# A-SHOJAEI/preference-guided-image-captioning-alignment

Measured on AMD Instinct MI355X. Metric: DPO preference-pairs/sec, CLIP-ViT-B/32+GPT-2-M seq128, higher is better.
Workload: dtype bf16; 1 GPU; Stage-2 DPO step, 4-forward policy/reference x chosen/rejected, openai/clip-vit-base-patch32 (frozen) + gpt2-medium decoder, seq_len 128, beta 0.1, bf16 MFMA / f32 accumulate+master, AdamW+clip; pairs_per_gpu=512, seq_len=128, parallelism=dp1, grad_allreduce=none (1 GPU)

## Files before the change

include/pgca_hip.h:

```cpp
#ifndef PGCA_HIP_H
#define PGCA_HIP_H

#include <stddef.h>
#include <stdint.h>

#ifdef __cplusplus
extern "C" {
#endif

typedef enum pgca_status {
  PGCA_OK = 0,
  PGCA_ERR_INVALID = -1,
  PGCA_ERR_LAUNCH = -2
} pgca_status;

#define PGCA_ABI_VERSION 306
int pgca_version(void);
int pgca_sizeof_gemm_args(void);
const char* pgca_last_error(void);

enum { PGCA_NT = 0, PGCA_NN = 1, PGCA_TN = 2 };

enum {
  PGCA_EPI_NONE = 0,
// ... 20 lines not shown
  int32_t epilogue;
  float alpha;
  const float* bias;
  void* out_bf16;
  int32_t ld_out_bf16;
  float* out_f32;
  int32_t ld_out_f32;
  int32_t accumulate;
  const float* residual;
  int32_t ld_res;
  void* aux_out;
  const void* aux_in;
  int32_t ld_aux;
  const int64_t* targets;
  float* stat_max;
  float* stat_sum;
  int32_t stat_ld;
  float* target_val;
  const float* row_lse;
  const float* row_scale;
  int32_t out_cols;
  uint32_t drop_seed;
  uint32_t drop_threshold;
  float drop_scale;
  float* colsum_part;
  int32_t ld_colsum;
  const int32_t* drop_rows;
} pgca_gemm_args;

int pgca_gemm_bf16(const pgca_gemm_args* args, void* stream);
int pgca_gemm_plan(const pgca_gemm_args* args);
int pgca_set_option(const char* name, int32_t value);
int pgca_gemm_bf16_grouped(const pgca_gemm_args* args, int32_t count, void* stream);

#define PGCA_SKINNY_MAX_M 64
typedef struct pgca_skinny_args {
  const void* x;
  const void* W;
  int32_t M, N, K, lda, ldw;
  float* scratch;
  const float* bias;
  int32_t act;
  const float* residual;
  int32_t ld_res;
  float* out_f32;
  int32_t ld_out_f32;
  void* out_bf16;
  int32_t ld_out_bf16;
  const float* ln_gamma;
  const float* ln_beta;
  float ln_eps;
  void* ln_out_bf16;
  int32_t ld_ln;
} pgca_skinny_args;
int pgca_gemm_skinny(const pgca_skinny_args* args, void* stream);
int64_t pgca_gemm_skinny_workspace(int32_t M, int32_t N, int32_t K);
int pgca_sizeof_skinny_args(void);

int pgca_rowstats_combine(const float* stat_max, const float* stat_sum, int32_t stat_ld, int32_t nparts,
                          const float* target_val, int32_t M, float* lse, float* out_logprob, void* stream);

int pgca_layernorm_fwd(const float* x, const int32_t* row_map, int32_t M, int32_t H, const float* gamma,
                       const float* beta, float eps, void* y_bf16, float* y_f32, float* mean, float* rstd,
                       void* stream);

int pgca_layernorm_bwd_blocks(int32_t M);
// ... 134 lines not shown
```

preference-guided-image-captioning-alignment_amd/csrc/gemm.hip:

```cpp
#include <string>

#include "gemm_device.h"

namespace {

template <int LA, int LB>
__global__ __launch_bounds__(256, 2) void gemm_kernel(const pgca_gemm_args a, int ntm, int ntn) {
  __shared__ __attribute__((aligned(16))) unsigned char smem[2][2][TILE_BYTES];

  int tm, tn;
  group_m_tile(xcd_remap(blockIdx.x, ntm * ntn), ntm, ntn, tm, tn);
  const int m0 = tm * BM, n0 = tn * BN;

  const int t = threadIdx.x;
  const int lane = t & 63, wave = t >> 6;
  const int wm = wave >> 1, wn = wave & 1;

  const bf16_t* A = reinterpret_cast<const bf16_t*>(a.A);
  const bf16_t* B = reinterpret_cast<const bf16_t*>(a.B);

  Stage<LA> sa;
  Stage<LB> sb;
  sa.init(t, a.lda, m0, LA == 0 ? a.M : ((a.M + 7) & ~7));
  sb.init(t, a.ldb, n0, LB == 0 ? a.N : ((a.N + 7) & ~7));
  const bf16_t* abase = LA == 0 ? A + (size_t)m0 * a.lda : A + m0;
  const bf16_t* bbase = LB == 0 ? B + (size_t)n0 * a.ldb : B + n0;
  const size_t astep = LA == 0 ? (size_t)BK : (size_t)BK * a.lda;
  const size_t bstep = LB == 0 ? (size_t)BK : (size_t)BK * a.ldb;

  f32x4 acc[4][4];
#pragma unroll
  for (int i = 0; i < 4; ++i)
#pragma unroll
    for (int j = 0; j < 4; ++j) acc[i][j] = (f32x4){0.f, 0.f, 0.f, 0.f};

// ... 27 lines not shown
        for (int j = 0; j < 4; ++j)
          acc[i][j] = __builtin_amdgcn_mfma_f32_16x16x32_bf16(fa[i], fb[j], acc[i][j], 0, 0, 0);
    }
    if (more) {
      sa.store(smem[cur ^ 1][0], ra);
      sb.store(smem[cur ^ 1][1], rb);
    }
    __syncthreads();
  }

  run_epilogue(a, acc, &smem[0][0][0], m0 + wm * 64, n0 + wn * 64, lane, wave);
}

__global__ void rowstats_combine_kernel(const float* __restrict__ smax, const float* __restrict__ ssum, int stat_ld,
                                        int nparts, const float* __restrict__ tval, int M, float* __restrict__ lse,
                                        float* __restrict__ out_lp) {
  const int row = blockIdx.x * (blockDim.x >> 6) + (threadIdx.x >> 6);
  const int lane = threadIdx.x & 63;
  if (row >= M) return;
  float mx = -INFINITY;
  for (int i = lane; i < nparts; i += 64) mx = fmaxf(mx, smax[(size_t)row * stat_ld + i]);
  mx = wave_max(mx);
  float s = 0.f;
  for (int i = lane; i < nparts; i += 64) {
    const float pm = smax[(size_t)row * stat_ld + i];
    if (pm > -INFINITY) s += ssum[(size_t)row * stat_ld + i] * __expf(pm - mx);
  }
  s = wave_sum(s);
  if (lane == 0) {
    const float l = mx + __logf(s);
    if (lse) lse[row] = l;
    if (out_lp) out_lp[row] = tval[row] - l;
  }
}


template <int LA, int LB, bool RAW = false>
__device__ __forceinline__ void gemm256_body(const pgca_gemm_args& a, int ntm, int ntn, int nk_per_split, int bid_in,
                                             int ksplit, unsigned char* smem2) {
  int tm, tn;
  if (RAW) {
    tm = bid_in / ntn;
    tn = bid_in - tm * ntn;
  } else {
    group_m_tile(xcd_remap(bid_in, ntm * ntn), ntm, ntn, tm, tn);
  }
  const int m0 = tm * BM2, n0 = tn * BN2;

  const int t = threadIdx.x;
  const int lane = t & 63;
  const int wave = __builtin_amdgcn_readfirstlane(t >> 6);
  const int wm = wave >> 2, wn = wave & 3;

  const bf16_t* A = reinterpret_cast<const bf16_t*>(a.A);
  const bf16_t* B = reinterpret_cast<const bf16_t*>(a.B);

  Dma<LA, BK> da;
  Dma<LB, BK> db;
  da.init(lane, wave, a.lda, m0, LA == 0 ? a.M : ((a.M + 7) & ~7));
  db.init(lane, wave, a.ldb, n0, LB == 0 ? a.N : ((a.N + 7) & ~7));
  const bf16_t* abase = LA == 0 ? A + (size_t)m0 * a.lda : A + m0;
  const bf16_t* bbase = LB == 0 ? B + (size_t)n0 * a.ldb : B + n0;
  const size_t astep = LA == 0 ? (size_t)BK : (size_t)BK * a.lda;
  const size_t bstep = LB == 0 ? (size_t)BK : (size_t)BK * a.ldb;

  f32x4 acc[2][4][4];
#pragma unroll
  for (int h = 0; h < 2; ++h)
#pragma unroll
    for (int i = 0; i < 4; ++i)
#pragma unroll
      for (int j = 0; j < 4; ++j) acc[h][i][j] = (f32x4){0.f, 0.f, 0.f, 0.f};

  const int kt0 = ksplit * nk_per_split;
  const int nk = min(nk_per_split, a.K / BK - kt0);
  abase += (size_t)kt0 * astep;
  bbase += (size_t)kt0 * bstep;
#ifdef PGCA_GEMM_TIMING
  unsigned long long ts0, ts1, ts2, ts3;
#endif
  TSTAMP(ts0);
  da.issue(abase, smem2, wave);
  db.issue(bbase, smem2 + TILE2_BYTES, wave);
  dma_wait();
  __syncthreads();
  TSTAMP(ts1);

  for (int kt = 0; kt < nk; ++kt) {
    const int cur = kt & 1;
    if (kt + 1 < nk) {
      unsigned char* nxt = smem2 + (cur ^ 1) * 2 * TILE2_BYTES;
      da.issue(abase + (size_t)(kt + 1) * astep, nxt, wave);
      db.issue(bbase + (size_t)(kt + 1) * bstep, nxt + TILE2_BYTES, wave);
    }
    const unsigned char* la = smem2 + cur * 2 * TILE2_BYTES;
    const unsigned char* lb = la + TILE2_BYTES;
#pragma unroll
    for (int kk = 0; kk < 2; ++kk) {
      bf16x8 fb[4];
#pragma unroll
      for (int j = 0; j < 4; ++j) fb[j] = read_frag<LB, 512>(lb, wn * 64, j, kk, lane);
      mma_half<LA>(la, wm * 128, kk, lane, fb, acc[0]);
      mma_half<LA>(la, wm * 128 + 64, kk, lane, fb, acc[1]);
    }
    dma_wait();
    __syncthreads();
  }

  TSTAMP(ts2);
  run_epilogue(a, acc[0], smem2, m0 + wm * 128, n0 + wn * 64, lane, wave);
  run_epilogue(a, acc[1], smem2, m0 + wm * 128 + 64, n0 + wn * 64, lane, wave);
#ifdef PGCA_GEMM_TIMING
  dma_wait();
  TSTAMP(ts3);
  if (a.stat_max && a.epilogue != PGCA_EPI_ROWSTATS && lane == 0) {
    float* o = a.stat_max + ((size_t)blockIdx.x * 8 + wave) * 8;
    o[0] = (float)(ts1 - ts0); o[1] = (float)(ts2 - ts1); o[2] = (float)(ts3 - ts2); o[3] = (float)nk;
  }
#endif
}

template <int LA, int LB>
__global__ __launch_bounds__(512, 2) void gemm256_kernel(const pgca_gemm_args a, int ntm, int ntn, int nk_per_split) {
  extern __shared__ __attribute__((aligned(16))) unsigned char smem2[];
  gemm256_body<LA, LB>(a, ntm, ntn, nk_per_split, blockIdx.x, blockIdx.y, smem2);
}

struct pgca_group_param {
  pgca_gemm_args a[4];
  int start[5];
  int ntm[4], ntn[4];
};

__global__ __launch_bounds__(512, 2) void gemm256_group_tn_kernel(const pgca_group_param gp) {
  extern __shared__ __attribute__((aligned(16))) unsigned char smem2[];
  const int b = xcd_remap(blockIdx.x, gp.start[4]);
  int p = 0;
  if (b >= gp.start[1]) p = 1;
  if (b >= gp.start[2]) p = 2;
  if (b >= gp.start[3]) p = 3;
#define PGCA_SEL(F) (p == 0 ? gp.a[0].F : p == 1 ? gp.a[1].F : p == 2 ? gp.a[2].F : gp.a[3].F)
  pgca_gemm_args a = {};
  a.A = PGCA_SEL(A);
  a.B = PGCA_SEL(B);
  a.M = PGCA_SEL(M);
  a.N = PGCA_SEL(N);
  a.K = PGCA_SEL(K);
  a.lda = PGCA_SEL(lda);
  a.ldb = PGCA_SEL(ldb);
  a.out_f32 = PGCA_SEL(out_f32);
  a.ld_out_f32 = PGCA_SEL(ld_out_f32);
  a.alpha = PGCA_SEL(alpha);
  a.accumulate = PGCA_SEL(accumulate);
  a.layout = PGCA_TN;
  a.epilogue = PGCA_EPI_NONE;
#undef PGCA_SEL
  const int ntm = p == 0 ? gp.ntm[0] : p == 1 ? gp.ntm[1] : p == 2 ? gp.ntm[2] : gp.ntm[3];
  const int ntn = p == 0 ? gp.ntn[0] : p == 1 ? gp.ntn[1] : p == 2 ? gp.ntn[2] : gp.ntn[3];
  const int st = p == 0 ? gp.start[0] : p == 1 ? gp.start[1] : p == 2 ? gp.start[2] : gp.start[3];
  const int l = b - st;
  int tm, tn;
  if (ntm <= ntn) {
    tn = l / ntm;
    tm = l - tn * ntm;
  } else {
    tm = l / ntn;
    tn = l - tm * ntn;
  }
  gemm256_body<1, 1, true>(a, ntm, ntn, a.K / BK, tm * ntn + tn, 0, smem2);
}

constexpr size_t GEMM256_LDS = 4 * TILE2_BYTES;

int plan_variant(const pgca_gemm_args& a) {
  const int forced = gemm_tuning().schedule;
  if (forced >= 0) return forced == 6 ? 6 : 0;
  return a.layout == PGCA_TN ? 0 : 6;
}

}

namespace pgca {
GemmTuning& gemm_tuning() {
  static GemmTuning t = [] {
    auto env = [](const char* name, int dflt) {
      const char* e = getenv(name);
      return e ? atoi(e) : dflt;
    };
    GemmTuning v;
    v.tile = env("PGCA_GEMM_TILE", 0);
    v.schedule = env("PGCA_GEMM_RING", -1);
    v.group = env("PGCA_GEMM_NO_GROUP", 0) ? 0 : 1;
    v.stagger = env("PGCA_GEMM_STAGGER", 0);
    v.pair_order = 0;
    return v;
  }();
  return t;
}

GemmPlan plan_gemm(const pgca_gemm_args& a) {
  GemmPlan p;
  p.ncols = a.epilogue == PGCA_EPI_DLOGITS ? a.out_cols : a.N;
  const int ntm2 = (a.M + BM2 - 1) / BM2, ntn2 = (p.ncols + BN2 - 1) / BN2;
  const int force = gemm_tuning().tile;
  const int nk_total = a.K / BK;
  int splits = 1;
// ... 151 lines not shown
    const pgca_gemm_args& a = args[i];
    groupable = a.layout == PGCA_TN && (a.K % BK) == 0 && a.M >= 8 && a.N >= 8 && a.epilogue == PGCA_EPI_NONE &&
                a.out_f32 && !a.out_bf16 && !a.bias && !a.residual && !a.drop_threshold &&
                check_gemm_args(a) == PGCA_OK;
  }
  if (!groupable) {
    for (int i = 0; i < count; ++i) {
      const int rc = pgca_gemm_bf16(&args[i], stream);
      if (rc) return rc;
    }
    return PGCA_OK;
  }
  if (raise_lds_limit<gemm256_group_tn_kernel>(GEMM256_LDS, "gemm256")) return PGCA_ERR_LAUNCH;
  pgca_group_param gp;
  int total = 0;
  for (int i = 0; i < 4; ++i) {
    if (i < count) {
      gp.a[i] = args[i];
      gp.ntm[i] = (args[i].M + BM2 - 1) / BM2;
      gp.ntn[i] = (args[i].N + BN2 - 1) / BN2;
      gp.start[i] = total;
      total += gp.ntm[i] * gp.ntn[i];
    } else {
      gp.a[i] = args[count - 1];
      gp.ntm[i] = gp.ntn[i] = 1;
      gp.start[i] = 0x7fffffff;
    }
  }
  gp.start[4] = total;
  hipLaunchKernelGGL(gemm256_group_tn_kernel, dim3(total), dim3(512), GEMM256_LDS, (hipStream_t)stream, gp);
  return check_launch("pgca_gemm_bf16_grouped");
}

extern "C" int pgca_rowstats_combine(const float* stat_max, const float* stat_sum, int32_t stat_ld, int32_t nparts,
                                     const float* target_val, int32_t M, float* lse, float* out_logprob,
                                     void* stream) {
  if (!stat_max || !stat_sum || M <= 0 || nparts <= 0 || (out_logprob && !target_val)) {
    set_error("pgca_rowstats_combine: bad arguments");
    return PGCA_ERR_INVALID;
  }
  hipLaunchKernelGGL(rowstats_combine_kernel, dim3((M + 3) / 4), dim3(256), 0, (hipStream_t)stream, stat_max,
                     stat_sum, stat_ld, nparts, target_val, M, lse, out_logprob);
  return check_launch("pgca_rowstats_combine");
}
```

preference-guided-image-captioning-alignment_amd/csrc/gemm_device.h:

```cpp
#pragma once
#include <stdlib.h>

#include <type_traits>

#include "common.h"

namespace pgca {
struct GemmPlan {
  int tile;
  int variant;
  int splits;
  int ntm, ntn;
  int nk_per_split;
  int grid_y;
  int ncols;
};
GemmPlan plan_gemm(const pgca_gemm_args& a);
int launch_gemm256s(const pgca_gemm_args& a, const GemmPlan& p, void* stream);
int launch_gemm256s_pair(const pgca_gemm_args& a0, const pgca_gemm_args& a1, const GemmPlan& p, void* stream);

struct GemmTuning {
  int tile;
  int schedule;
  int group;
  int pair_order;
  int stagger;
};
GemmTuning& gemm_tuning();
}

using namespace pgca;

namespace {

template <typename F>
int with_layout(int layout, F&& f) {
  using S0 = std::integral_constant<int, 0>;
  using S1 = std::integral_constant<int, 1>;
  switch (layout) {
    case PGCA_NT: return f(S0{}, S0{});
    case PGCA_NN: return f(S0{}, S1{});
    case PGCA_TN: return f(S1{}, S1{});
    default: set_error("pgca_gemm_bf16: unknown layout %d", layout); return PGCA_ERR_INVALID;
  }
}

template <auto KERNEL>
int raise_lds_limit(size_t bytes, const char* what) {
  static const bool ok = hipFuncSetAttribute((const void*)KERNEL, hipFuncAttributeMaxDynamicSharedMemorySize,
                                             (int)bytes) == hipSuccess;
  if (!ok) {
    (void)hipGetLastError();
// ... 178 lines not shown
```

preference-guided-image-captioning-alignment_amd/csrc/gemm_pair.hip:

```cpp
#include "gemm_phase_body.h"

namespace {

struct pgca_pair_param {
  pgca_gemm_args a[2];
  int ntm, ntn, nk, stagger;
  int order;
};

template <int LA, int LB>
__global__ __launch_bounds__(512, 2) void gemm256s_pair_kernel(const pgca_pair_param gp) {
  extern __shared__ __attribute__((aligned(16))) unsigned char smems[];
  const int ntm = gp.ntm, ntn = gp.ntn, nwg = ntm * ntn;
  const int b = xcd_remap(blockIdx.x, 2 * nwg);
  int p, bid;
  if (gp.order == 0) {
    p = b >= nwg;
    bid = b - (p ? nwg : 0);
  } else {
    const int per_group = GROUP_M * ntn;
    const int g = b / (2 * per_group);
    const int size = min(GROUP_M, ntm - g * GROUP_M) * ntn;
    const int rem = b - g * 2 * per_group;
    p = rem >= size;
    bid = g * per_group + rem - (p ? size : 0);
  }
  p = __builtin_amdgcn_readfirstlane(p);
  bid = __builtin_amdgcn_readfirstlane(bid);
  const char* kernarg = (const char*)__builtin_amdgcn_kernarg_segment_ptr();
  const pgca_gemm_args a = *(const pgca_gemm_args*)(kernarg + offsetof(pgca_pair_param, a) +
                                                    (p ? sizeof(pgca_gemm_args) : 0));
  if (a.epilogue > PGCA_EPI_TANH && a.epilogue != PGCA_EPI_GELU_NEW_D) return;
  gemm256s_body<LA, LB>(a, ntm, ntn, gp.nk, gp.stagger, bid, smems);
}

}

int pgca::launch_gemm256s_pair(const pgca_gemm_args& a0, const pgca_gemm_args& a1, const GemmPlan& p, void* stream) {
  auto forward_epilogue = [](int e) { return (e >= PGCA_EPI_NONE && e <= PGCA_EPI_TANH) || e == PGCA_EPI_GELU_NEW_D; };
  if (!forward_epilogue(a0.epilogue) || !forward_epilogue(a1.epilogue)) {
    const int rc = launch_gemm256s(a0, p, stream);
    return rc ? rc : launch_gemm256s(a1, p, stream);
  }
  pgca_pair_param gp;
  gp.a[0] = a0;
  gp.a[1] = a1;
  gp.ntm = p.ntm;
  gp.ntn = p.ntn;
  gp.nk = p.nk_per_split;
  gp.stagger = 2 * p.ntm * p.ntn >= 3 * 256 ? gemm_tuning().stagger : 0;
  gp.order = gemm_tuning().pair_order;
  auto launch = [&](auto lb) {
    constexpr auto kernel = gemm256s_pair_kernel<0, decltype(lb)::value>;
    if (raise_lds_limit<kernel>(GEMM256S_LDS, "gemm256s pair")) return (int)PGCA_ERR_LAUNCH;
    hipLaunchKernelGGL(kernel, dim3(2 * p.ntm * p.ntn), dim3(512), GEMM256S_LDS, (hipStream_t)stream, gp);
    return check_launch("pgca_gemm_bf16_grouped(256 phase-staggered pair)");
  };
  return a0.layout == PGCA_NT ? launch(std::integral_constant<int, 0>{}) : launch(std::integral_constant<int, 1>{});
}
```

preference-guided-image-captioning-alignment_amd/csrc/gemm_phase.hip:

```cpp
#include "gemm_phase_body.h"

namespace {

template <int LA, int LB>
__global__ __launch_bounds__(512, 2) void gemm256s_kernel(const pgca_gemm_args a, int ntm, int ntn, int nk_per_split,
                                                          int stagger) {
  extern __shared__ __attribute__((aligned(16))) unsigned char smems[];
  gemm256s_body<LA, LB>(a, ntm, ntn, nk_per_split, stagger, xcd_remap(blockIdx.x, ntm * ntn), smems);
}

}

int pgca::launch_gemm256s(const pgca_gemm_args& a, const GemmPlan& p, void* stream) {
  return with_layout(a.layout, [&](auto la, auto lb) {
    constexpr auto kernel = gemm256s_kernel<decltype(la)::value, decltype(lb)::value>;
    if (raise_lds_limit<kernel>(GEMM256S_LDS, "gemm256s")) return (int)PGCA_ERR_LAUNCH;
    const int stagger = (p.ntm * p.ntn >= 3 * 256 && p.grid_y == 1) ? gemm_tuning().stagger : 0;
    hipLaunchKernelGGL(kernel, dim3(p.ntm * p.ntn, p.grid_y), dim3(512), GEMM256S_LDS, (hipStream_t)stream, a, p.ntm,
                       p.ntn, p.nk_per_split, stagger);
    return check_launch("pgca_gemm_bf16(256 phase-staggered)");
  });
}
```

preference-guided-image-captioning-alignment_amd/csrc/gemm_phase_body.h:

```cpp
#pragma once
#include <stddef.h>

#include "gemm_device.h"

namespace {

constexpr int PBK = 32, PSTAGES = 4;
constexpr int PTILE_BYTES = 256 * PBK * 2;

template <int KS>
using DmaP = Dma<KS, PBK>;

template <int KS>
__device__ __forceinline__ bf16x8 read_frag_p(const unsigned char* lds, int wbase, int sub, int lane) {
  if (KS == 0) {
    const int row = wbase + sub * 16 + (lane & 15);
    const int pos = (lane >> 4) ^ swz4p((lane >> 2) & 3);
    return *reinterpret_cast<const bf16x8*>(lds + row * 64 + pos * 16);
  } else {
    return read_frag<1, 512>(lds, wbase, sub, 0, lane);
  }
}


template <int N>
__device__ __forceinline__ void wait_vm_p() {
  asm volatile("s_waitcnt vmcnt(%0)" ::"n"(N) : "memory");
}

#ifndef PGCA_FILL_L
#define PGCA_FILL_L 0
#endif
#ifndef PGCA_FILL_M
#define PGCA_FILL_M 0
#endif
template <int N>
__device__ __forceinline__ void valu_fill(float (&d)[8]) {
#pragma unroll
  for (int i = 0; i < N; ++i) asm volatile("v_fmac_f32 %0, %1, %1" : "+v"(d[i & 7]) : "v"(d[(i + 3) & 7]));
}
#define PGCA_PBAR()                       \
  do {                                    \
    __builtin_amdgcn_sched_barrier(0);    \
    __builtin_amdgcn_s_barrier();         \
    __builtin_amdgcn_sched_barrier(0);    \
  } while (0)

template <int LA, int LB>
__device__ __forceinline__ void gemm256s_body(const pgca_gemm_args& a, int ntm, int ntn, int nk_per_split, int stagger,
                                              int bid, unsigned char* smems) {
#ifdef PGCA_GEMM_TIMING
  unsigned long long ts0, ts1, ts2, ts3, tr0, tr3;
#endif
  TSTAMP(ts0);
  TSTAMP_REAL(tr0);

  if (stagger > 0 && gridDim.y == 1 && blockIdx.x < 256) {
    const int slot = (blockIdx.x >> 3) & 3;
    for (int i = 0; i < slot * stagger; ++i) __builtin_amdgcn_s_sleep(16);
  }

  int tm, tn;
  group_m_tile(bid, ntm, ntn, tm, tn);
  const int m0 = tm * BM2, n0 = tn * BN2;

  const int t = threadIdx.x;
  const int lane = t & 63;
  const int wave = __builtin_amdgcn_readfirstlane(t >> 6);
  const int wm = wave >> 2, wn = wave & 3;

  const bf16_t* A = reinterpret_cast<const bf16_t*>(a.A);
  const bf16_t* B = reinterpret_cast<const bf16_t*>(a.B);

  DmaP<LA> da;
  DmaP<LB> db;
  da.init(lane, wave, a.lda, m0, LA == 0 ? a.M : ((a.M + 7) & ~7));
  db.init(lane, wave, a.ldb, n0, LB == 0 ? a.N : ((a.N + 7) & ~7));
  const bf16_t* abase = LA == 0 ? A + (size_t)m0 * a.lda : A + m0;
  const bf16_t* bbase = LB == 0 ? B + (size_t)n0 * a.ldb : B + n0;
  const size_t astep = LA == 0 ? (size_t)PBK : (size_t)PBK * a.lda;
  const size_t bstep = LB == 0 ? (size_t)PBK : (size_t)PBK * a.ldb;

  f32x4 acc[2][4][4];
#pragma unroll
  for (int h = 0; h < 2; ++h)
#pragma unroll
    for (int i = 0; i < 4; ++i)
#pragma unroll
      for (int j = 0; j < 4; ++j) acc[h][i][j] = (f32x4){0.f, 0.f, 0.f, 0.f};

  const int kt0 = blockIdx.y * nk_per_split * 2;
  const int nk = min(nk_per_split * 2, a.K / PBK - kt0);
  abase += (size_t)kt0 * astep;
  bbase += (size_t)kt0 * bstep;

  da.issue(abase, smems, wave);
  db.issue(bbase, smems + PTILE_BYTES, wave);
  da.issue(abase + astep, smems + 2 * PTILE_BYTES, wave);
  db.issue(bbase + bstep, smems + 3 * PTILE_BYTES, wave);
  if (2 < nk) {
    da.issue(abase + 2 * astep, smems + 4 * PTILE_BYTES, wave);
    wait_vm_p<6>();
  } else {
    wait_vm_p<4>();
  }
  PGCA_PBAR();
  PGCA_PBAR();
  if (wm == 1) PGCA_PBAR();

  TSTAMP(ts1);
#ifdef PGCA_GEMM_TIMING2
  unsigned long long q0 = 0, q1 = 0, q2 = 0, q3 = 0, q4 = 0, q5 = 0, q6 = 0, q7 = 0, q8 = 0;
  unsigned long long aL0 = 0, aB1 = 0, aM0 = 0, aB2 = 0, aL1 = 0, aB3 = 0, aM1 = 0, aB4 = 0;
#endif
  float fill[8] = {1.f, 2.f, 3.f, 4.f, 5.f, 6.f, 7.f, 8.f};
  for (int kt = 0; kt < nk; ++kt) {
    PSTAMP(q0);
    const unsigned char* la = smems + (kt & 3) * 2 * PTILE_BYTES;
    const unsigned char* lb = la + PTILE_BYTES;
    bf16x8 fa[4], fb[4];
#pragma unroll
    for (int j = 0; j < 4; ++j) fb[j] = read_frag_p<LB>(lb, wn * 64, j, lane);
#pragma unroll
    for (int i = 0; i < 4; ++i) fa[i] = read_frag_p<LA>(la, wm * 128, i, lane);
// ... 89 lines not shown
```

preference-guided-image-captioning-alignment_amd/engine.py:

```python
from __future__ import annotations

import logging
import math
import os
from contextlib import contextmanager
from dataclasses import dataclass
from types import SimpleNamespace
from typing import Dict, List, Optional, Tuple

import torch

from . import hip
from .arch import GptArch, ModelArch, VitArch
from .params import ParamStore, Segment, VOCAB_TILE

logger = logging.getLogger(__name__)

F32, BF16, I32, I64 = torch.float32, torch.bfloat16, torch.int32, torch.int64
ATTN_BWD_MAX_S = 1024
ATTN_BWD_ONEPASS_MAX_S = 512


def attention_backward(qkv, out, dout, lse, key_mask, B, S, heads, causal, dqkv, drop=None, cu=None):
    fn = hip.attention_bwd if S <= ATTN_BWD_ONEPASS_MAX_S else hip.attention_bwd_split
# ... 1004 lines not shown
            torch.cuda.synchronize()
        return out

    def decode_reorder(self, src: torch.Tensor) -> None:
        self.trunk.decode_reorder(self._dec, src)

    def _decode_logits(self, x: torch.Tensor) -> torch.Tensor:
        a, st = self.arch.gpt, self._dec
        R, H = st.R, a.hidden
        self.trunk.decode_step(x, st, st.t)
        if st.lnf_done:
            hf = self.trunk._buf("gen.y", (R, H), BF16)
        else:
            hf = self._buf("gen.hf", (R, H), BF16)
            hip.layernorm_fwd(x, R, H, self.trunk.lnf_w.w, self.trunk.lnf_b.w, a.eps, y_bf16=hf)
        ldv = (self.V + 3) // 4 * 4
        out = self._buf("gen.logits", (R, ldv), F32)
        hip.gemm(hf, self.wte.b, R, self.V, H, hip.NT, out_f32=out, ld_out_f32=ldv)
        return out[:, :self.V]

    def backward(self, dseq: torch.Tensor) -> torch.Tensor:
        s = self.saved
        sb: SeqBatch = s["sb"]
        a = self.arch.gpt
        H, Pd, Bq, S, Mc = a.hidden, self.arch.proj_dim, sb.Bq, sb.S, sb.n_rows
        pack: Optional[RowPack] = s["pack"]
        rw = _rows(pack, Bq, S)
        M = rw.M
        ws = self.ws
        rs = self._buf("row_scale", (Mc,), F32)
        hip.row_scale(dseq, sb.seq_of_row, sb.counts, Mc, (1 if s["reduce"] == "mean" else 0) | 2, rs)
        dhf = self._buf("dhf32", (Mc, H), F32, zero=True)
        ck = min(self.LM_CHUNK, Mc)
        dl = self._buf("dlogits", (ck, self.Vp), BF16)
        for r0 in range(0, Mc, ck):
            n = min(ck, Mc - r0)
            hfc = s["hf"][r0:r0 + n]
            hip.gemm(hfc, self.wte.b, n, self.V, H, hip.NT, epilogue=hip.EPI_DLOGITS, targets=sb.targets[r0:r0 + n],
                     row_lse=s["lse"][r0:r0 + n], row_scale=rs[r0:r0 + n], out_bf16=dl, ld_out_bf16=self.Vp,
                     out_cols=self.Vp)
            hip.gemm(dl, self.wte_pad_bf, n, H, self.Vp, hip.NN, lda=self.Vp, ldb=H, out_f32=dhf[r0:r0 + n], accumulate=True)
            hip.gemm(dl, hfc, self.V, H, n, hip.TN, lda=self.Vp, ldb=H, out_f32=self.wte.g, accumulate=True)
        g = self.trunk._buf("g_top", (M, H), F32, zero=True)
        g_bf = self.trunk._buf("gbf_top", (M, H), BF16, zero=True)
        nb = hip.layernorm_bwd_blocks(Mc)
        part = ws.get("ln_part_f", (2, nb, H), F32)
        hip.layernorm_bwd(s["hL"], Mc, H, self.trunk.lnf_w.w, s["mf"], s["rf"], g, dy_f32=dhf,
                          row_map=sb.row_map_packed if pack is not None else sb.row_map, dx_bf16=g_bf, part=part,
                          drop_dx=self.trunk.top_drop(), drop_rows=rw.ids)
        _ln_param_grads(part, nb, H, self.trunk.lnf_w.g, self.trunk.lnf_b.g)
        g0 = self.trunk.backward(g, g_bf)
        drop = s["drop"]
        XH = self.arch.xattn_heads
        dh = H // XH
        datt = self._buf("datt", (Bq, H), F32, zero=True)
        nbe = hip.embed_bwd_blocks(Bq, S)
        parte = ws.get("ln_part_e", (2, nbe, H), F32)
        dvv = self._buf("dvv", (Bq, H), BF16)
        if drop is None:
            hip.embed_bwd(g0, sb.ids, sb.mask, Bq, S, H, self.wte.g, self.wpe.g, wte=self.wte.w, attended=s["att"],
                          gamma=self.anw.w, mean=s["m0"], rstd=s["r0"], dattended=datt, part=parte, cu=rw.cu)
            _ln_param_grads(parte, nbe, H, self.anw.g, self.anb.g)
            datt_bf = self._buf("datt_bf", (Bq, H), BF16)
            hip.cast_bf16(datt, datt_bf, Bq * H)
            hip.gemm(datt_bf, s["vv"], H, H, Bq, hip.TN, lda=H, ldb=H, out_f32=self.ow.g, accumulate=True)
            _bias_grad(ws, Bq, H, H, self.ob.g, x_f32=datt)
            hip.gemm(datt_bf, self.ow.b, Bq, H, H, hip.NN, out_bf16=dvv)
        else:
            dU = self._buf("dU", (Bq, XH, H), F32, zero=True)
            hip.embed_bwd(g0, sb.ids, sb.mask, Bq, S, H, self.wte.g, self.wpe.g, wte=self.wte.w, attended=self.ob.w,
                          att_stride=0, gamma=self.anw.w, mean=s["m0"], rstd=s["r0"], dattended=datt, part=parte,
                          U=s["U"], dU=dU, xheads=XH, drop_x=drop(0, KIND_XATTN), drop_e=drop(0, KIND_EMBD), cu=rw.cu)
            _ln_param_grads(parte, nbe, H, self.anw.g, self.anb.g)
            _bias_grad(ws, Bq, H, H, self.ob.g, x_f32=datt)
            dU_bf = self._buf("dU_bf", (Bq, XH, H), BF16)
# ... 180 lines not shown
```

preference-guided-image-captioning-alignment_amd/hip.py:

```python
from __future__ import annotations

import ctypes as C
import os
from typing import Optional

import torch

_HERE = os.path.dirname(os.path.abspath(__file__))
LIB_PATH = os.environ.get("PGCA_LIB") or os.path.join(_HERE, "libpgca_hip.so")

NT, NN, TN = 0, 1, 2
EPI_NONE, EPI_GELU_NEW, EPI_QUICK_GELU, EPI_RELU, EPI_TANH = 0, 1, 2, 3, 4
EPI_DGELU_NEW, EPI_DRELU, EPI_DTANH, EPI_ROWSTATS, EPI_DLOGITS, EPI_DQUICK_GELU = 5, 6, 7, 8, 9, 10
EPI_GELU_NEW_D, EPI_MUL_AUX = 11, 12

_vp, _i32, _i64, _f32 = C.c_void_p, C.c_int32, C.c_int64, C.c_float


class GemmArgs(C.Structure):
    _fields_ = [
        ("A", _vp), ("B", _vp),
        ("M", _i32), ("N", _i32), ("K", _i32),
        ("lda", _i32), ("ldb", _i32),
        ("layout", _i32), ("epilogue", _i32),
# ... 7 lines not shown
        ("targets", _vp), ("stat_max", _vp), ("stat_sum", _vp), ("stat_ld", _i32),
        ("target_val", _vp), ("row_lse", _vp), ("row_scale", _vp),
        ("out_cols", _i32),
        ("drop_seed", C.c_uint32), ("drop_threshold", C.c_uint32), ("drop_scale", _f32),
        ("colsum_part", _vp), ("ld_colsum", _i32),
        ("drop_rows", _vp),
    ]


class SkinnyArgs(C.Structure):
    _fields_ = [
        ("x", _vp), ("W", _vp),
        ("M", _i32), ("N", _i32), ("K", _i32), ("lda", _i32), ("ldw", _i32),
        ("scratch", _vp), ("bias", _vp), ("act", _i32),
        ("residual", _vp), ("ld_res", _i32),
        ("out_f32", _vp), ("ld_out_f32", _i32),
        ("out_bf16", _vp), ("ld_out_bf16", _i32),
        ("ln_gamma", _vp), ("ln_beta", _vp), ("ln_eps", _f32),
        ("ln_out_bf16", _vp), ("ld_ln", _i32),
    ]


class SelectOpts(C.Structure):
    _fields_ = [("no_repeat_ngram_size", _i32), ("n_ban", _i32), ("ban_ids", _vp)]


SKINNY_MAX_M = 64

_SIGS = {
    "pgca_gemm_bf16": [C.POINTER(GemmArgs), _vp],
    "pgca_gemm_plan": [C.POINTER(GemmArgs)],
    "pgca_set_option": [C.c_char_p, _i32],
    "pgca_gemm_bf16_grouped": [C.POINTER(GemmArgs), _i32, _vp],
    "pgca_gemm_skinny": [C.POINTER(SkinnyArgs), _vp],
    "pgca_rowstats_combine": [_vp, _vp, _i32, _i32, _vp, _i32, _vp, _vp, _vp],
    "pgca_layernorm_fwd": [_vp, _vp, _i32, _i32, _vp, _vp, _f32, _vp, _vp, _vp, _vp, _vp],
    "pgca_layernorm_bwd_blocks": [_i32],
    "pgca_layernorm_bwd": [_vp, _vp, _vp, _vp, _i32, _i32, _vp, _vp, _vp, _vp, _vp, _vp, _vp, _vp, _vp, _vp, _vp, _vp],
    "pgca_colsum_finish": [_vp, _i32, _i32, _vp, _i32, _vp],
    "pgca_colsum_finish4": [_vp, _i32, _i32, _i32, _vp, _vp, _vp, _vp, _i32, _vp],
    "pgca_colsum_blocks": [_i32],
    "pgca_colsum": [_vp, _vp, _i32, _i32, _i32, _vp, _vp],
    "pgca_attention_fwd": [_vp, _vp, _i32, _i32, _i32, _i32, _vp, _vp, C.c_uint32, C.c_uint32, _f32, _vp, _vp],
    "pgca_attention_bwd": [_vp, _vp, _vp, _vp, _vp, _i32, _i32, _i32, _i32, _vp, C.c_uint32, C.c_uint32, _f32, _vp, _vp],
    "pgca_attention_bwd_split": [_vp, _vp, _vp, _vp, _vp, _i32, _i32, _i32, _i32, _vp, C.c_uint32, C.c_uint32, _f32, _vp,
                                 _vp],
    "pgca_embed_fwd": [_vp, _i32, _i32, _i32, _vp, _vp, _vp, _vp, _vp, _f32, _vp, _vp, _vp, _i32, _vp, _i32, _vp, _vp,
                       _vp, _i32, _vp],
    "pgca_embed_bwd": [_vp, _vp, _vp, _i32, _i32, _i32, _vp, _vp, _vp, _vp, _vp, _vp, _vp, _vp, _vp, _i32, _vp, _vp,
                       _i32, _vp, _vp, _vp, _vp],
    "pgca_embed_bwd_blocks": [_i32, _i32],
    "pgca_patchify": [_vp, _i32, _i32, _i32, _i32, _vp, _vp],
    "pgca_image_preprocess": [_vp, _i32, _i32, _i32, _i32, _vp, _vp, _i32, _vp, _vp, _i32, _f32, _f32, _f32, _f32, _f32, _f32,
                              _vp, _vp, _vp, _vp],
    "pgca_image_train_transform": [_vp, _i32, _i32, _i32, _i32, _vp, _vp, _vp, _vp, _i32, _vp, _vp, _i32, _f32, _f32, _f32,
                                   _f32, _f32, _f32, _vp, _vp, _vp, _vp, _vp],
    "pgca_vit_assemble": [_vp, _vp, _vp, _i32, _i32, _i32, _vp, _vp],
    "pgca_vit_assemble_bwd": [_vp, _i32, _i32, _i32, _vp, _vp, _vp, _vp],
    "pgca_seq_reduce": [_vp, _vp, _i32, _i32, _vp, _i32, _vp, _vp],
    "pgca_logits_logprob": [_vp, _i32, _i32, _vp, _vp, _i32, _vp, _vp],
    "pgca_logits_logprob_bwd": [_vp, _i32, _i32, _vp, _vp, _vp, _i32, _vp, _vp],
    "pgca_dpo_loss": [_vp, _vp, _vp, _vp, _i32, _f32, _f32, _vp, _vp, _vp, _vp, _vp],
    "pgca_row_scale": [_vp, _vp, _vp, _i32, _i32, _vp, _vp],
    "pgca_seq_batch_prepare": [_vp, _vp, _i32, _i32, _vp, _vp, _vp, _vp, _vp, _vp, _vp],
    "pgca_seq_pack_prepare": [_vp, _i32, _i32, _i32, _vp, _vp, _vp, _vp, _vp, _vp, _vp],
    "pgca_masked_mean_fwd": [_vp, _vp, _i32, _i32, _i32, _vp, _vp, _vp],
# ... 124 lines not shown
        probe, e0, e1 = bracket
        e1.record()
        probe.add(e0, e1, flops)


def gemm(A: torch.Tensor, B: torch.Tensor, M: int, N: int, K: int, layout: int, **kw) -> None:
    a = _gemm_args(A, B, M, N, K, layout, **kw)
    bracket = _probe_begin(a)
    _check(load().pgca_gemm_bf16(C.byref(a), _stream()), "pgca_gemm_bf16")
    _probe_end(bracket, 2.0 * M * N * K)


def gemm_pair(g0, g1) -> None:
    arr = (GemmArgs * 2)()
    for a, (args, kw) in zip(arr, (g0, g1)):
        _gemm_args(*args, **kw, into=a)
    bracket = _probe_begin(arr[0])
    _check(load().pgca_gemm_bf16_grouped(arr, 2, _stream()), "pgca_gemm_bf16_grouped")
    _probe_end(bracket, sum(2.0 * a.M * a.N * a.K for a in arr))


def _wgrad_group_args(problems):
    arr = (GemmArgs * len(problems))()
    for a, (X, dY, M, N, K, gout) in zip(arr, problems):
        _gemm_args(X, dY, M, N, K, TN, out_f32=gout, accumulate=True, into=a)
    return arr


def gemm_wgrad_group(problems) -> None:
    _check(load().pgca_gemm_bf16_grouped(_wgrad_group_args(problems), len(problems), _stream()),
           "pgca_gemm_bf16_grouped")


def gemm_skinny(x, W, M, N, K, scratch, *, lda=None, ldw=None, bias=None, act=EPI_NONE, residual=None, ld_res=None,
                out_f32=None, ld_out_f32=None, out_bf16=None, ld_out_bf16=None, ln=None, ln_out=None, ld_ln=None):
    a = SkinnyArgs()
    a.x, a.W = x.data_ptr(), W.data_ptr()
    a.M, a.N, a.K = M, N, K
    a.lda, a.ldw = (K if lda is None else lda), (N if ldw is None else ldw)
    a.scratch, a.bias, a.act = scratch.data_ptr(), _p(bias), act
    a.residual, a.ld_res = _p(residual), (N if ld_res is None else ld_res)
    a.out_f32, a.ld_out_f32 = _p(out_f32), (N if ld_out_f32 is None else ld_out_f32)
    a.out_bf16, a.ld_out_bf16 = _p(out_bf16), (N if ld_out_bf16 is None else ld_out_bf16)
    if ln is not None:
        a.ln_gamma, a.ln_beta, a.ln_eps = ln[0].data_ptr(), ln[1].data_ptr(), float(ln[2])
        a.ln_out_bf16, a.ld_ln = ln_out.data_ptr(), (N if ld_ln is None else ld_ln)
    _check(load().pgca_gemm_skinny(C.byref(a), _stream()), "pgca_gemm_skinny")


def gemm_skinny_workspace(M: int, N: int, K: int) -> int:
    return int(load().pgca_gemm_skinny_workspace(M, N, K))


def drop_args(seed: int, p: float):
    if p <= 0.0:
        return None
    return (seed & 0xFFFFFFFF, min(0xFFFFFFFF, int(p * 4294967296.0)), 1.0 / (1.0 - p))


def set_option(name: str, value: int) -> None:
    _check(load().pgca_set_option(name.encode(), int(value)), "pgca_set_option")


gemm_probe = None


# ... 265 lines not shown
```

Before: 2007 pairs/s.

## Group LM-head backward GEMMs with next chunk's dlogits in one launch

Adds a grouped kernel that runs, in a single launch, the LM-head weight-gradient GEMM and data-gradient GEMM for the current vocab-logit chunk together with the dlogits GEMM for the next chunk, using double-buffered dlogits buffers. The aim is to fill the GPU better and cut the launch and tail gaps between the three serial GEMMs per chunk. It adds a second dlogits buffer and falls back to separate launches when the plans do not match the expected tile/variant. Correctness relies on the wgrad and dgrad blocks of chunk c only reading dlogits buffer c&1 while the next chunk's dlogits GEMM writes the other buffer.

```diff
diff --git a/include/pgca_hip.h b/include/pgca_hip.h
--- a/include/pgca_hip.h
+++ b/include/pgca_hip.h
@@ -76,6 +76,8 @@
 int pgca_gemm_plan(const pgca_gemm_args* args);
 int pgca_set_option(const char* name, int32_t value);
 int pgca_gemm_bf16_grouped(const pgca_gemm_args* args, int32_t count, void* stream);
+int pgca_lm_head_bwd_group(const pgca_gemm_args* wgrad, const pgca_gemm_args* dgrad, const pgca_gemm_args* dlogits,
+                           int32_t* grouped, void* stream);
 
 #define PGCA_SKINNY_MAX_M 64
 typedef struct pgca_skinny_args {
diff --git a/preference-guided-image-captioning-alignment_amd/csrc/gemm.hip b/preference-guided-image-captioning-alignment_amd/csrc/gemm.hip
--- a/preference-guided-image-captioning-alignment_amd/csrc/gemm.hip
+++ b/preference-guided-image-captioning-alignment_amd/csrc/gemm.hip
@@ -1,6 +1,6 @@
 #include <string>
 
-#include "gemm_device.h"
+#include "gemm256_body.h"
 
 namespace {
 
@@ -94,92 +94,6 @@
     if (lse) lse[row] = l;
     if (out_lp) out_lp[row] = tval[row] - l;
   }
-}
-
-
-template <int LA, int LB, bool RAW = false>
-__device__ __forceinline__ void gemm256_body(const pgca_gemm_args& a, int ntm, int ntn, int nk_per_split, int bid_in,
-                                             int ksplit, unsigned char* smem2) {
-  int tm, tn;
-  if (RAW) {
-    tm = bid_in / ntn;
-    tn = bid_in - tm * ntn;
-  } else {
-    group_m_tile(xcd_remap(bid_in, ntm * ntn), ntm, ntn, tm, tn);
-  }
-  const int m0 = tm * BM2, n0 = tn * BN2;
-
-  const int t = threadIdx.x;
-  const int lane = t & 63;
-  const int wave = __builtin_amdgcn_readfirstlane(t >> 6);
-  const int wm = wave >> 2, wn = wave & 3;
-
-  const bf16_t* A = reinterpret_cast<const bf16_t*>(a.A);
-  const bf16_t* B = reinterpret_cast<const bf16_t*>(a.B);
-
-  Dma<LA, BK> da;
-  Dma<LB, BK> db;
-  da.init(lane, wave, a.lda, m0, LA == 0 ? a.M : ((a.M + 7) & ~7));
-  db.init(lane, wave, a.ldb, n0, LB == 0 ? a.N : ((a.N + 7) & ~7));
-  const bf16_t* abase = LA == 0 ? A + (size_t)m0 * a.lda : A + m0;
-  const bf16_t* bbase = LB == 0 ? B + (size_t)n0 * a.ldb : B + n0;
-  const size_t astep = LA == 0 ? (size_t)BK : (size_t)BK * a.lda;
-  const size_t bstep = LB == 0 ? (size_t)BK : (size_t)BK * a.ldb;
-
-  f32x4 acc[2][4][4];
-#pragma unroll
-  for (int h = 0; h < 2; ++h)
-#pragma unroll
-    for (int i = 0; i < 4; ++i)
-#pragma unroll
-      for (int j = 0; j < 4; ++j) acc[h][i][j] = (f32x4){0.f, 0.f, 0.f, 0.f};
-
-  const int kt0 = ksplit * nk_per_split;
-  const int nk = min(nk_per_split, a.K / BK - kt0);
-  abase += (size_t)kt0 * astep;
-  bbase += (size_t)kt0 * bstep;
-#ifdef PGCA_GEMM_TIMING
-  unsigned long long ts0, ts1, ts2, ts3;
-#endif
-  TSTAMP(ts0);
-  da.issue(abase, smem2, wave);
-  db.issue(bbase, smem2 + TILE2_BYTES, wave);
-  dma_wait();
-  __syncthreads();
-  TSTAMP(ts1);
-
-  for (int kt = 0; kt < nk; ++kt) {
-    const int cur = kt & 1;
-    if (kt + 1 < nk) {
-      unsigned char* nxt = smem2 + (cur ^ 1) * 2 * TILE2_BYTES;
-      da.issue(abase + (size_t)(kt + 1) * astep, nxt, wave);
-      db.issue(bbase + (size_t)(kt + 1) * bstep, nxt + TILE2_BYTES, wave);
-    }
-    const unsigned char* la = smem2 + cur * 2 * TILE2_BYTES;
-    const unsigned char* lb = la + TILE2_BYTES;
-#pragma unroll
-    for (int kk = 0; kk < 2; ++kk) {
-      bf16x8 fb[4];
-#pragma unroll
-      for (int j = 0; j < 4; ++j) fb[j] = read_frag<LB, 512>(lb, wn * 64, j, kk, lane);
-      mma_half<LA>(la, wm * 128, kk, lane, fb, acc[0]);
-      mma_half<LA>(la, wm * 128 + 64, kk, lane, fb, acc[1]);
-    }
-    dma_wait();
-    __syncthreads();
-  }
-
-  TSTAMP(ts2);
-  run_epilogue(a, acc[0], smem2, m0 + wm * 128, n0 + wn * 64, lane, wave);
-  run_epilogue(a, acc[1], smem2, m0 + wm * 128 + 64, n0 + wn * 64, lane, wave);
-#ifdef PGCA_GEMM_TIMING
-  dma_wait();
-  TSTAMP(ts3);
-  if (a.stat_max && a.epilogue != PGCA_EPI_ROWSTATS && lane == 0) {
-    float* o = a.stat_max + ((size_t)blockIdx.x * 8 + wave) * 8;
-    o[0] = (float)(ts1 - ts0); o[1] = (float)(ts2 - ts1); o[2] = (float)(ts3 - ts2); o[3] = (float)nk;
-  }
-#endif
 }
 
 template <int LA, int LB>
@@ -232,8 +146,6 @@
   gemm256_body<1, 1, true>(a, ntm, ntn, a.K / BK, tm * ntn + tn, 0, smem2);
 }
 
-constexpr size_t GEMM256_LDS = 4 * TILE2_BYTES;
-
 int plan_variant(const pgca_gemm_args& a) {
   const int forced = gemm_tuning().schedule;
   if (forced >= 0) return forced == 6 ? 6 : 0;
@@ -451,6 +363,48 @@
   return check_launch("pgca_gemm_bf16_grouped");
 }
 
+extern "C" int pgca_lm_head_bwd_group(const pgca_gemm_args* wgrad, const pgca_gemm_args* dgrad,
+                                      const pgca_gemm_args* dlogits, int32_t* grouped, void* stream) {
+  if (grouped) *grouped = 0;
+  if (!wgrad || !dgrad) {
+    set_error("pgca_lm_head_bwd_group: the weight-gradient and data-gradient problems are required");
+    return PGCA_ERR_INVALID;
+  }
+  const pgca_gemm_args* all[3] = {wgrad, dgrad, dlogits};
+  for (const pgca_gemm_args* a : all)
+    if (a)
+      if (const int rc = check_gemm_args(*a)) return rc;
+  auto plain_f32 = [](const pgca_gemm_args& a) {
+    return a.epilogue == PGCA_EPI_NONE && a.out_f32 && a.accumulate && !a.out_bf16 && !a.bias && !a.residual &&
+           !a.aux_out && !a.aux_in && !a.colsum_part && !a.drop_threshold;
+  };
+  bool group = gemm_tuning().group && wgrad->layout == PGCA_TN && plain_f32(*wgrad) && dgrad->layout == PGCA_NN &&
+               plain_f32(*dgrad);
+  if (group && dlogits)
+    group = dlogits->layout == PGCA_NT && dlogits->epilogue == PGCA_EPI_DLOGITS && !dlogits->out_f32 && !dlogits->bias &&
+            !dlogits->residual && !dlogits->aux_out && !dlogits->aux_in && !dlogits->colsum_part &&
+            !dlogits->drop_threshold;
+  GemmPlan pw{}, pd{}, pl{};
+  if (group) {
+    pw = plan_gemm(*wgrad);
+    pd = plan_gemm(*dgrad);
+    group = pw.tile == 256 && pw.variant == 0 && pw.splits == 1 && pd.tile == 256 && pd.variant == 6;
+    if (group && dlogits) {
+      pl = plan_gemm(*dlogits);
+      group = pl.tile == 256 && pl.variant == 6 && pl.splits == 1;
+    }
+  }
+  if (!group) {
+    for (const pgca_gemm_args* a : all)
+      if (a)
+        if (const int rc = pgca_gemm_bf16(a, stream)) return rc;
+    return PGCA_OK;
+  }
+  if (const int rc = launch_lm_head_group(*dgrad, pd, *wgrad, pw, dlogits, pl, stream)) return rc;
+  if (grouped) *grouped = 1;
+  return PGCA_OK;
+}
+
 extern "C" int pgca_rowstats_combine(const float* stat_max, const float* stat_sum, int32_t stat_ld, int32_t nparts,
                                      const float* target_val, int32_t M, float* lse, float* out_logprob,
                                      void* stream) {
diff --git a/preference-guided-image-captioning-alignment_amd/csrc/gemm256_body.h b/preference-guided-image-captioning-alignment_amd/csrc/gemm256_body.h
--- /dev/null
+++ b/preference-guided-image-captioning-alignment_amd/csrc/gemm256_body.h
@@ -0,0 +1,93 @@
+#pragma once
+#include "gemm_device.h"
+
+namespace {
+
+template <int LA, int LB, bool RAW = false>
+__device__ __forceinline__ void gemm256_body(const pgca_gemm_args& a, int ntm, int ntn, int nk_per_split, int bid_in,
+                                             int ksplit, unsigned char* smem2) {
+  int tm, tn;
+  if (RAW) {
+    tm = bid_in / ntn;
+    tn = bid_in - tm * ntn;
+  } else {
+    group_m_tile(xcd_remap(bid_in, ntm * ntn), ntm, ntn, tm, tn);
+  }
+  const int m0 = tm * BM2, n0 = tn * BN2;
+
+  const int t = threadIdx.x;
+  const int lane = t & 63;
+  const int wave = __builtin_amdgcn_readfirstlane(t >> 6);
+  const int wm = wave >> 2, wn = wave & 3;
+
+  const bf16_t* A = reinterpret_cast<const bf16_t*>(a.A);
+  const bf16_t* B = reinterpret_cast<const bf16_t*>(a.B);
+
+  Dma<LA, BK> da;
+  Dma<LB, BK> db;
+  da.init(lane, wave, a.lda, m0, LA == 0 ? a.M : ((a.M + 7) & ~7));
+  db.init(lane, wave, a.ldb, n0, LB == 0 ? a.N : ((a.N + 7) & ~7));
+  const bf16_t* abase = LA == 0 ? A + (size_t)m0 * a.lda : A + m0;
+  const bf16_t* bbase = LB == 0 ? B + (size_t)n0 * a.ldb : B + n0;
+  const size_t astep = LA == 0 ? (size_t)BK : (size_t)BK * a.lda;
+  const size_t bstep = LB == 0 ? (size_t)BK : (size_t)BK * a.ldb;
+
+  f32x4 acc[2][4][4];
+#pragma unroll
+  for (int h = 0; h < 2; ++h)
+#pragma unroll
+    for (int i = 0; i < 4; ++i)
+#pragma unroll
+      for (int j = 0; j < 4; ++j) acc[h][i][j] = (f32x4){0.f, 0.f, 0.f, 0.f};
+
+  const int kt0 = ksplit * nk_per_split;
+  const int nk = min(nk_per_split, a.K / BK - kt0);
+  abase += (size_t)kt0 * astep;
+  bbase += (size_t)kt0 * bstep;
+#ifdef PGCA_GEMM_TIMING
+  unsigned long long ts0, ts1, ts2, ts3;
+#endif
+  TSTAMP(ts0);
+  da.issue(abase, smem2, wave);
+  db.issue(bbase, smem2 + TILE2_BYTES, wave);
+  dma_wait();
+  __syncthreads();
+  TSTAMP(ts1);
+
+  for (int kt = 0; kt < nk; ++kt) {
+    const int cur = kt & 1;
+    if (kt + 1 < nk) {
+      unsigned char* nxt = smem2 + (cur ^ 1) * 2 * TILE2_BYTES;
+      da.issue(abase + (size_t)(kt + 1) * astep, nxt, wave);
+      db.issue(bbase + (size_t)(kt + 1) * bstep, nxt + TILE2_BYTES, wave);
+    }
+    const unsigned char* la = smem2 + cur * 2 * TILE2_BYTES;
+    const unsigned char* lb = la + TILE2_BYTES;
+#pragma unroll
+    for (int kk = 0; kk < 2; ++kk) {
+      bf16x8 fb[4];
+#pragma unroll
+      for (int j = 0; j < 4; ++j) fb[j] = read_frag<LB, 512>(lb, wn * 64, j, kk, lane);
+      mma_half<LA>(la, wm * 128, kk, lane, fb, acc[0]);
+      mma_half<LA>(la, wm * 128 + 64, kk, lane, fb, acc[1]);
+    }
+    dma_wait();
+    __syncthreads();
+  }
+
+  TSTAMP(ts2);
+  run_epilogue(a, acc[0], smem2, m0 + wm * 128, n0 + wn * 64, lane, wave);
+  run_epilogue(a, acc[1], smem2, m0 + wm * 128 + 64, n0 + wn * 64, lane, wave);
+#ifdef PGCA_GEMM_TIMING
+  dma_wait();
+  TSTAMP(ts3);
+  if (a.stat_max && a.epilogue != PGCA_EPI_ROWSTATS && lane == 0) {
+    float* o = a.stat_max + ((size_t)blockIdx.x * 8 + wave) * 8;
+    o[0] = (float)(ts1 - ts0); o[1] = (float)(ts2 - ts1); o[2] = (float)(ts3 - ts2); o[3] = (float)nk;
+  }
+#endif
+}
+
+constexpr size_t GEMM256_LDS = 4 * TILE2_BYTES;
+
+}
diff --git a/preference-guided-image-captioning-alignment_amd/csrc/gemm_device.h b/preference-guided-image-captioning-alignment_amd/csrc/gemm_device.h
--- a/preference-guided-image-captioning-alignment_amd/csrc/gemm_device.h
+++ b/preference-guided-image-captioning-alignment_amd/csrc/gemm_device.h
@@ -18,6 +18,8 @@
 GemmPlan plan_gemm(const pgca_gemm_args& a);
 int launch_gemm256s(const pgca_gemm_args& a, const GemmPlan& p, void* stream);
 int launch_gemm256s_pair(const pgca_gemm_args& a0, const pgca_gemm_args& a1, const GemmPlan& p, void* stream);
+int launch_lm_head_group(const pgca_gemm_args& dgrad, const GemmPlan& pd, const pgca_gemm_args& wgrad, const GemmPlan& pw,
+                         const pgca_gemm_args* dlogits, const GemmPlan& pl, void* stream);
 
 struct GemmTuning {
   int tile;
diff --git a/preference-guided-image-captioning-alignment_amd/csrc/gemm_lm_group.hip b/preference-guided-image-captioning-alignment_amd/csrc/gemm_lm_group.hip
--- /dev/null
+++ b/preference-guided-image-captioning-alignment_amd/csrc/gemm_lm_group.hip
@@ -0,0 +1,77 @@
+#include "gemm256_body.h"
+#include "gemm_phase_body.h"
+
+namespace {
+
+static_assert(GEMM256_LDS == GEMM256S_LDS, "both main loops use the whole 128 KiB");
+
+struct pgca_lm_group_param {
+  pgca_gemm_args a[3];
+  int end[3];
+  int ntm[3], ntn[3];
+  int nk[3];
+};
+
+__device__ __forceinline__ pgca_gemm_args plain_f32_args(pgca_gemm_args a) {
+  a.epilogue = PGCA_EPI_NONE;
+  a.bias = nullptr;
+  a.out_bf16 = nullptr;
+  a.residual = nullptr;
+  a.aux_out = nullptr;
+  a.aux_in = nullptr;
+  a.colsum_part = nullptr;
+  a.drop_threshold = 0;
+  return a;
+}
+
+__global__ __launch_bounds__(512, 2) void lm_head_bwd_group_kernel(const pgca_lm_group_param gp) {
+  extern __shared__ __attribute__((aligned(16))) unsigned char smem[];
+  const int b = blockIdx.x;
+  if (b < gp.end[0]) {
+    const pgca_gemm_args a = plain_f32_args(gp.a[0]);
+    const int nt = gp.ntm[0] * gp.ntn[0];
+    const int ks = __builtin_amdgcn_readfirstlane(b / nt);
+    gemm256s_body<0, 1>(a, gp.ntm[0], gp.ntn[0], gp.nk[0], 0, xcd_remap(b - ks * nt, nt), ks, smem);
+  } else if (b < gp.end[1]) {
+    pgca_gemm_args a = plain_f32_args(gp.a[1]);
+    a.accumulate = 1;
+    gemm256_body<1, 1>(a, gp.ntm[1], gp.ntn[1], gp.nk[1], b - gp.end[0], 0, smem);
+  } else {
+    pgca_gemm_args a = gp.a[2];
+    a.epilogue = PGCA_EPI_DLOGITS;
+    a.bias = nullptr;
+    a.out_f32 = nullptr;
+    a.residual = nullptr;
+    a.aux_out = nullptr;
+    a.aux_in = nullptr;
+    a.colsum_part = nullptr;
+    a.drop_threshold = 0;
+    a.accumulate = 0;
+    const int nt = gp.ntm[2] * gp.ntn[2];
+    gemm256s_body<0, 0>(a, gp.ntm[2], gp.ntn[2], gp.nk[2], 0, xcd_remap(b - gp.end[1], nt), 0, smem);
+  }
+}
+
+}
+
+int pgca::launch_lm_head_group(const pgca_gemm_args& dgrad, const GemmPlan& pd, const pgca_gemm_args& wgrad,
+                               const GemmPlan& pw, const pgca_gemm_args* dlogits, const GemmPlan& pl, void* stream) {
+  pgca_lm_group_param gp;
+  gp.a[0] = dgrad;
+  if (pd.splits > 1) gp.a[0].accumulate = 2;
+  gp.a[1] = wgrad;
+  gp.a[2] = dlogits ? *dlogits : wgrad;
+  const GemmPlan* plans[3] = {&pd, &pw, &pl};
+  int total = 0;
+  for (int p = 0; p < 3; ++p) {
+    const bool present = p < 2 || dlogits;
+    gp.ntm[p] = present ? plans[p]->ntm : 1;
+    gp.ntn[p] = present ? plans[p]->ntn : 1;
+    gp.nk[p] = present ? plans[p]->nk_per_split : 1;
+    if (present) total += plans[p]->ntm * plans[p]->ntn * plans[p]->grid_y;
+    gp.end[p] = total;
+  }
+  if (raise_lds_limit<lm_head_bwd_group_kernel>(GEMM256S_LDS, "lm_head_bwd_group")) return PGCA_ERR_LAUNCH;
+  hipLaunchKernelGGL(lm_head_bwd_group_kernel, dim3(total), dim3(512), GEMM256S_LDS, (hipStream_t)stream, gp);
+  return check_launch("pgca_lm_head_bwd_group");
+}
diff --git a/preference-guided-image-captioning-alignment_amd/csrc/gemm_pair.hip b/preference-guided-image-captioning-alignment_amd/csrc/gemm_pair.hip
--- a/preference-guided-image-captioning-alignment_amd/csrc/gemm_pair.hip
+++ b/preference-guided-image-captioning-alignment_amd/csrc/gemm_pair.hip
@@ -31,7 +31,7 @@
   const pgca_gemm_args a = *(const pgca_gemm_args*)(kernarg + offsetof(pgca_pair_param, a) +
                                                     (p ? sizeof(pgca_gemm_args) : 0));
   if (a.epilogue > PGCA_EPI_TANH && a.epilogue != PGCA_EPI_GELU_NEW_D) return;
-  gemm256s_body<LA, LB>(a, ntm, ntn, gp.nk, gp.stagger, bid, smems);
+  gemm256s_body<LA, LB>(a, ntm, ntn, gp.nk, gp.stagger, bid, 0, smems);
 }
 
 }
diff --git a/preference-guided-image-captioning-alignment_amd/csrc/gemm_phase.hip b/preference-guided-image-captioning-alignment_amd/csrc/gemm_phase.hip
--- a/preference-guided-image-captioning-alignment_amd/csrc/gemm_phase.hip
+++ b/preference-guided-image-captioning-alignment_amd/csrc/gemm_phase.hip
@@ -6,7 +6,7 @@
 __global__ __launch_bounds__(512, 2) void gemm256s_kernel(const pgca_gemm_args a, int ntm, int ntn, int nk_per_split,
                                                           int stagger) {
   extern __shared__ __attribute__((aligned(16))) unsigned char smems[];
-  gemm256s_body<LA, LB>(a, ntm, ntn, nk_per_split, stagger, xcd_remap(blockIdx.x, ntm * ntn), smems);
+  gemm256s_body<LA, LB>(a, ntm, ntn, nk_per_split, stagger, xcd_remap(blockIdx.x, ntm * ntn), blockIdx.y, smems);
 }
 
 }
diff --git a/preference-guided-image-captioning-alignment_amd/csrc/gemm_phase_body.h b/preference-guided-image-captioning-alignment_amd/csrc/gemm_phase_body.h
--- a/preference-guided-image-captioning-alignment_amd/csrc/gemm_phase_body.h
+++ b/preference-guided-image-captioning-alignment_amd/csrc/gemm_phase_body.h
@@ -48,7 +48,7 @@
 
 template <int LA, int LB>
 __device__ __forceinline__ void gemm256s_body(const pgca_gemm_args& a, int ntm, int ntn, int nk_per_split, int stagger,
-                                              int bid, unsigned char* smems) {
+                                              int bid, int ksplit, unsigned char* smems) {
 #ifdef PGCA_GEMM_TIMING
   unsigned long long ts0, ts1, ts2, ts3, tr0, tr3;
 #endif
@@ -89,7 +89,7 @@
 #pragma unroll
       for (int j = 0; j < 4; ++j) acc[h][i][j] = (f32x4){0.f, 0.f, 0.f, 0.f};
 
-  const int kt0 = blockIdx.y * nk_per_split * 2;
+  const int kt0 = ksplit * nk_per_split * 2;
   const int nk = min(nk_per_split * 2, a.K / PBK - kt0);
   abase += (size_t)kt0 * astep;
   bbase += (size_t)kt0 * bstep;
diff --git a/preference-guided-image-captioning-alignment_amd/engine.py b/preference-guided-image-captioning-alignment_amd/engine.py
--- a/preference-guided-image-captioning-alignment_amd/engine.py
+++ b/preference-guided-image-captioning-alignment_amd/engine.py
@@ -1060,15 +1060,30 @@
         hip.row_scale(dseq, sb.seq_of_row, sb.counts, Mc, (1 if s["reduce"] == "mean" else 0) | 2, rs)
         dhf = self._buf("dhf32", (Mc, H), F32, zero=True)
         ck = min(self.LM_CHUNK, Mc)
-        dl = self._buf("dlogits", (ck, self.Vp), BF16)
-        for r0 in range(0, Mc, ck):
+        dls = [self._buf("dlogits", (ck, self.Vp), BF16)]
+        if Mc > ck:
+            dls.append(self._buf("dlogits1", (ck, self.Vp), BF16))
+
+        def dlogits_gemm(c):
+            r0 = c * ck
             n = min(ck, Mc - r0)
-            hfc = s["hf"][r0:r0 + n]
-            hip.gemm(hfc, self.wte.b, n, self.V, H, hip.NT, epilogue=hip.EPI_DLOGITS, targets=sb.targets[r0:r0 + n],
-                     row_lse=s["lse"][r0:r0 + n], row_scale=rs[r0:r0 + n], out_bf16=dl, ld_out_bf16=self.Vp,
-                     out_cols=self.Vp)
-            hip.gemm(dl, self.wte_pad_bf, n, H, self.Vp, hip.NN, lda=self.Vp, ldb=H, out_f32=dhf[r0:r0 + n], accumulate=True)
-            hip.gemm(dl, hfc, self.V, H, n, hip.TN, lda=self.Vp, ldb=H, out_f32=self.wte.g, accumulate=True)
+            return ((s["hf"][r0:r0 + n], self.wte.b, n, self.V, H, hip.NT),
+                    dict(epilogue=hip.EPI_DLOGITS, targets=sb.targets[r0:r0 + n], row_lse=s["lse"][r0:r0 + n],
+                         row_scale=rs[r0:r0 + n], out_bf16=dls[c & 1], ld_out_bf16=self.Vp, out_cols=self.Vp))
+
+        nchunks = (Mc + ck - 1) // ck
+        first = dlogits_gemm(0)
+        hip.gemm(*first[0], **first[1])
+        for c in range(nchunks):
+            r0 = c * ck
+            n = min(ck, Mc - r0)
+            dl = dls[c & 1]
+            hip.lm_head_bwd_group(
+                ((dl, s["hf"][r0:r0 + n], self.V, H, n, hip.TN),
+                 dict(lda=self.Vp, ldb=H, out_f32=self.wte.g, accumulate=True)),
+                ((dl, self.wte_pad_bf, n, H, self.Vp, hip.NN),
+                 dict(lda=self.Vp, ldb=H, out_f32=dhf[r0:r0 + n], accumulate=True)),
+                dlogits_gemm(c + 1) if c + 1 < nchunks else None)
         g = self.trunk._buf("g_top", (M, H), F32, zero=True)
         g_bf = self.trunk._buf("gbf_top", (M, H), BF16, zero=True)
         nb = hip.layernorm_bwd_blocks(Mc)
diff --git a/preference-guided-image-captioning-alignment_amd/hip.py b/preference-guided-image-captioning-alignment_amd/hip.py
--- a/preference-guided-image-captioning-alignment_amd/hip.py
+++ b/preference-guided-image-captioning-alignment_amd/hip.py
@@ -63,6 +63,7 @@
     "pgca_gemm_plan": [C.POINTER(GemmArgs)],
     "pgca_set_option": [C.c_char_p, _i32],
     "pgca_gemm_bf16_grouped": [C.POINTER(GemmArgs), _i32, _vp],
+    "pgca_lm_head_bwd_group": [C.POINTER(GemmArgs), C.POINTER(GemmArgs), C.POINTER(GemmArgs), C.POINTER(_i32), _vp],
     "pgca_gemm_skinny": [C.POINTER(SkinnyArgs), _vp],
     "pgca_rowstats_combine": [_vp, _vp, _i32, _i32, _vp, _i32, _vp, _vp, _vp],
     "pgca_layernorm_fwd": [_vp, _vp, _i32, _i32, _vp, _vp, _f32, _vp, _vp, _vp, _vp, _vp],
@@ -253,6 +254,17 @@
            "pgca_gemm_bf16_grouped")
 
 
+def lm_head_bwd_group(wgrad, dgrad, dlogits=None) -> bool:
+    arr = (GemmArgs * 3)()
+    for a, g in zip(arr, (wgrad, dgrad, dlogits)):
+        if g is not None:
+            _gemm_args(*g[0], **g[1], into=a)
+    grouped = _i32(0)
+    _check(load().pgca_lm_head_bwd_group(C.byref(arr[0]), C.byref(arr[1]), C.byref(arr[2]) if dlogits is not None else None,
+                                         C.byref(grouped), _stream()), "pgca_lm_head_bwd_group")
+    return bool(grouped.value)
+
+
 def gemm_skinny(x, W, M, N, K, scratch, *, lda=None, ldw=None, bias=None, act=EPI_NONE, residual=None, ld_res=None,
                 out_f32=None, ld_out_f32=None, out_bf16=None, ld_out_bf16=None, ln=None, ln_out=None, ld_ln=None):
     a = SkinnyArgs()
```

Measured after the change: 2028 pairs/s (median of 6 runs). 1.1% higher.
